# rvaser/rala

Measured on AMD Instinct MI355X. Metric: overlaps/sec (pile build + transitive reduction), higher is better.
Workload: dtype u16/u32 (+f64 compares)

## Files before the change

rala_amd/csrc/context.h:

```cpp
#pragma once

#include <hip/hip_runtime.h>
#include <stdint.h>

#include <algorithm>

#include <memory>
#include <string>
#include <vector>

#include "geom.h"
#include "host_pool.h"
#include "kernels.h"
#include "rala_hip.h"

namespace rala_hip {

struct HostOvl {
    uint32_t src;
    uint32_t a, b;
    Coords c;
    uint8_t strand;
    uint8_t dead;
    uint8_t type;
// ... 145 lines not shown
    hipStream_t side = nullptr;
    hipStream_t aux = nullptr;
    bool use_side_stream = true;
    std::string err;
    hipEvent_t ev[12] = {};
    hipStream_t copy = nullptr;
    hipEvent_t ev_up[4] = {};
    bool upload_pending = false, upload_queued = false;
    const uint32_t* up_src[7] = {};
    const uint8_t* up_strand = nullptr;

    int64_t pool_per_read_x1000 = 1000;
    int64_t max_lds_read_len = 22000;
    int64_t debug_pile_stop_after = 99;
    int64_t host_threads = 0;
    std::unique_ptr<rala_hip::HostPool> pool;
    bool use_run_kernel = true;
    bool debug_fail_construct = false;
    uint32_t debug_pile_variant = 0;
    uint32_t debug_dedupe_list_cap = 0;
    uint32_t debug_fp_lds_limit = 0xFFFFFFFFu;
    bool use_bound_records = true;
    bool use_round_batches = true;
    rala_hip::DevBuf<uint32_t> d_round_log;

    uint64_t n_reads = 0;
    uint32_t max_read_len = 0;
    uint32_t n_class[rala_hip::kPileClasses] = {};
    rala_hip::DevBuf<uint32_t> d_class_order;
    rala_hip::DevBuf<uint32_t> d_seg_base;
    rala_hip::DevBuf<uint32_t> d_dense;
    std::vector<uint32_t> h_read_len;
    std::vector<uint64_t> h_pile_off;
    uint64_t pile_elems = 0;
    rala_hip::DevBuf<uint32_t> d_read_len;
    rala_hip::DevBuf<uint64_t> d_pile_off;
    rala_hip::DevBuf<uint16_t> d_pile;
    rala_hip::DevBuf<uint32_t> d_order, d_overflow;
    rala_hip::DevBuf<uint32_t> d_big_list[2], d_big_space;
    int64_t debug_big_caps = 0;
    bool debug_force_big = false;
    rala_hip::DevBuf<uint16_t> d_slab;
    std::vector<rala_hip::LaunchClass> classes;

    rala_hip::DevBuf<uint8_t> d_name_buckets, d_name_arena, d_paf_text, d_paf_strand;
    uint64_t n_name_buckets = 0;
// ... 145 lines not shown
```

rala_amd/csrc/kernels.h:

```cpp
#pragma once

#include <hip/hip_runtime.h>
#include <stdint.h>

namespace rala_hip {

constexpr uint32_t kPadL = 848;

enum : uint32_t {
    kErrRegionCapacity = 1u,
    kErrPoolCapacity = 2u,
    kErrRawCapacity = 4u,
};

struct Interval {
    uint32_t first, second;
    uint32_t aux;
};

struct PileArgs {
    const uint32_t* read_len;
    const uint64_t* pile_off;
    uint16_t* pile;
    const uint32_t* ev_off;
// ... 222 lines not shown
    const uint32_t* ev_off;
    const uint32_t* ev_cnt;
    uint32_t ev_stride;
    uint32_t ev_shift;
    const uint32_t* sens_off;
    const uint32_t* begin;
    const uint32_t* end;
    uint32_t* out[5];
    uint32_t* counts;
};
void launch_sens_split(const uint32_t* list, uint32_t bound, const uint32_t* n_dev, const SensSplitArgs& args, hipStream_t s);
void launch_status_clear(uint32_t* status, uint32_t bits, uint32_t* zero, hipStream_t s);
void launch_scatter_component_medians(const uint32_t* alive_reads, const uint8_t* touched, const uint16_t* cmed, uint32_t n_alive,
                                      uint16_t* out, hipStream_t s);
void launch_break_hills(const TailReads& R, uint32_t n_reads, hipStream_t s);
void launch_break_pits(const TailReads& R, const uint32_t* alive_reads, const uint8_t* touched, const uint16_t* comp_median,
                       uint32_t n_alive, hipStream_t s, const uint32_t* gate = nullptr);
void launch_retrim(const TailList& L, const TailReads& R, uint32_t promote, uint32_t round, uint32_t* dropped,
                   hipStream_t s, const uint32_t* gate = nullptr);
void launch_cc_edges(const TailList& L, const uint32_t* rank, uint32_t* edges, uint8_t* touched, uint32_t* label, uint32_t n_labels,
                     hipStream_t s);
void launch_refresh_types(const TailList& L, const TailReads& R, hipStream_t s);
hipError_t launch_tail_contain(const TailList& L, const TailReads& R, uint8_t* alive, uint32_t* const lists[6], uint32_t* zeroed21, uint32_t* const work[4],
                               uint32_t* base2, uint8_t* mark2, uint32_t* map, uint32_t* pack, uint32_t n_reads, uint32_t lds_limit, hipStream_t s);
void launch_count_zero_u8(const uint8_t* x, uint32_t n, uint32_t* out, hipStream_t s);
void launch_tail_init(const TailList& L, uint32_t n0, const TailReads& R, uint32_t* n_pits0, uint32_t n_reads, uint32_t* base2,
                      uint8_t* mark2, uint32_t* map, uint32_t* zero22, hipStream_t s);
struct ScanSpace;
bool launch_rank_pass(const uint8_t* alive, uint32_t* rank, uint32_t* alive_reads, uint32_t n_reads, ScanSpace& space, hipStream_t s);
bool launch_node_pass(const uint8_t* alive, uint32_t* node_rank, uint32_t* node_read, uint32_t* n_final, uint32_t n_reads,
                      ScanSpace& space, hipStream_t s);
bool launch_segment_pass(const TailList& L, const TailReads& R, uint32_t want_state, uint32_t want_round, uint32_t* base,
                         uint32_t* next, uint32_t* kept_item, const uint32_t* node_rank, uint32_t* e_src, uint32_t* e_dst,
                         uint32_t* e_len, ScanSpace& space, hipStream_t s);
bool launch_offsets_pass(const uint32_t* in, uint32_t* out, uint32_t* copy, uint32_t n, ScanSpace& space, hipStream_t s);
bool launch_pair_offsets_pass(const uint32_t* in0, const uint32_t* in1, uint32_t* out0, uint32_t* out1, uint32_t* totals, uint32_t n,
                              ScanSpace& space, hipStream_t s);

struct FixedPointList {
    const uint32_t *key, *target, *keeper;
    const uint32_t* count;
    uint32_t lds_limit = 0xFFFFFFFFu;
    uint32_t debug_give_up = 0;
};
size_t fixed_point_pack_words();
hipError_t launch_fixed_point_finish(const FixedPointList& list, uint32_t* base, uint32_t* map, uint32_t* pack, uint32_t* const work[4],
                                     uint32_t* sync8, uint32_t* error, uint32_t* rounds_out, hipStream_t s);

struct FillList {
    static constexpr uint32_t kMost = 8;
    void* ptr[kMost];
    size_t bytes[kMost];
    uint8_t value[kMost];
    uint32_t n = 0;
    bool overflow = false;
    void add(void* p, int byte, size_t n_bytes);
    hipError_t launch(hipStream_t s);
// ... 100 lines not shown
```

rala_amd/csrc/pipeline.hip:

```cpp
#include <hip/hip_runtime.h>
#include <stdio.h>
#include <stdlib.h>
#include <string.h>

#include <algorithm>
#include <chrono>
#include <numeric>

#include "context.h"
#include "scan_pass.h"
#include "stages.h"

using namespace rala_hip;


hipError_t rala_hip::d2h_small(rala_hip_ctx* ctx, void* dst, const void* src, size_t bytes, hipStream_t s) {
    if (ctx->p_stage.ensure(256) != hipSuccess || ctx->stage_used + bytes > 256 * sizeof(uint32_t) ||
        ctx->stage_pending.size() >= 16) {
        return hipMemcpyAsync(dst, src, bytes, hipMemcpyDeviceToHost, s);
    }
    char* at = (char*)ctx->p_stage.p + ctx->stage_used;
    const hipError_t e = hipMemcpyAsync(at, src, bytes, hipMemcpyDeviceToHost, s);
    if (e != hipSuccess) return e;
    ctx->stage_pending.push_back({dst, ctx->stage_used, bytes});
// ... 713 lines not shown
        }
    }
    return true;
}

int materialize_host(rala_hip_ctx* ctx);
int download_repeat_hills(rala_hip_ctx* ctx) {
    if (!ctx->rep_host_stale) return RALA_HIP_OK;
    const uint64_t n = ctx->n_reads;
    HIPCHECK(hipSetDevice(ctx->device));
    ctx->h_n_rep.resize(n); ctx->h_rep_slot.resize(n);
    HIPCHECK(hipMemcpy(ctx->h_n_rep.data(), ctx->d_n_rep.p, n * 4, hipMemcpyDeviceToHost));
    HIPCHECK(hipMemcpy(ctx->h_rep_slot.data(), ctx->d_rep_slot.p, n * 4, hipMemcpyDeviceToHost));
    ctx->h_rep_pool.resize(ctx->n_rep_hills);
    if (ctx->n_rep_hills) {
        HIPCHECK(hipMemcpy(ctx->h_rep_pool.data(), ctx->d_rep_pool.p, (size_t)ctx->n_rep_hills * sizeof(Interval), hipMemcpyDeviceToHost));
    }
    ctx->rep_host_stale = false;
    return RALA_HIP_OK;
}
void build_graph(rala_hip_ctx* ctx);
TailList tail_list(rala_hip_ctx* ctx);
int tail_components(rala_hip_ctx* ctx, const TailList& L, uint32_t n_alive, bool touched_cleared = false);
int gpu_tail_part_b(rala_hip_ctx* ctx);

int preprocess_repeats(rala_hip_ctx* cs, rala_hip_ctx* cl, Comm* comm, const rala_hip_overlaps* sens, uint64_t n_sens,
                       bool device_lists) {
    rala_hip_ctx* ctx = cs;
    const bool sharded = comm != nullptr;
    const uint32_t P = sharded ? comm->world() : 1u, me = sharded ? comm->rank() : 0u;
    const uint64_t n = cs->n_reads;
    const uint64_t nl = cl->n_reads;
    const uint64_t nl_pad = ((n + P - 1) / P + 15) / 16 * 16;
    hipStream_t s = cs->stream;
    hipStream_t sl = cl->stream;
    Trace trc;
    auto comm_fail = [&](const char* what) {
        cs->err = std::string(what) + ": " + comm->error();
        cs->stage_pending.clear();
        cs->stage_used = 0;
        return RALA_HIP_EDEVICE;
    };
    if (n_sens >= 0x7FFFFFF0ull / 2) return fail(ctx, RALA_HIP_EINVAL, "too many sensitive overlaps");
    OvlSoA so;
    {
        const uint32_t* src[7] = {nullptr, nullptr, nullptr, nullptr, nullptr, nullptr, nullptr};
        const uint8_t* dev_strand = nullptr;
// ... 454 lines not shown
}

int tail_components(rala_hip_ctx* ctx, const TailList& L, uint32_t n_alive, bool touched_cleared) {
    hipStream_t s = ctx->stream;
    const uint32_t M = L.n;
    if (!touched_cleared) {
        FillList fills;
        fills.add(ctx->d_touched.p, 0, n_alive);
        component_median_clear(ctx->d_med_tmp.p, n_alive, fills);
        HIPCHECK(fills.launch(s));
    }
    launch_cc_edges(L, ctx->d_rank.p, ctx->d_cc_edges.p, ctx->d_touched.p, ctx->d_cc_label.p, n_alive, s);
    for (int k = 0; k < 2; ++k) {
        launch_cc_hook(ctx->d_cc_edges.p, M, 1, ctx->d_cc_label.p, ctx->d_cc_flags.p + 7, s);
        launch_cc_compress(ctx->d_cc_label.p, n_alive, s);
    }
    launch_cc_hook(ctx->d_cc_edges.p, M, 0, ctx->d_cc_label.p, ctx->d_cc_flags.p + 7, s);
    launch_cc_compress_count(ctx->d_cc_label.p, n_alive, ctx->d_touched.p, component_median_sizes(ctx->d_med_tmp.p, n_alive), s);
    HIPCHECK(launch_component_medians(ctx->d_cc_label.p, ctx->d_touched.p, ctx->d_alive_reads.p, ctx->d_median.p, n_alive,
                                      ctx->d_med_tmp.p, ctx->d_cmed.p, s));
    return RALA_HIP_OK;
}

int gpu_tail_part_a(rala_hip_ctx* ctx) {
    hipStream_t s = ctx->stream;
    Trace trc;
    auto mark = [&](const char* what, size_t k = 0) {
        if (trc.on) { (void)stream_sync(ctx, s); trc(what, k); }
    };
    const uint32_t n_reads = (uint32_t)ctx->n_reads;
    const uint32_t M = ctx->t_n0 + ctx->t_n1;
    const uint32_t n_alive = ctx->t_n_alive;
    const size_t big = (size_t)std::max<uint64_t>(n_reads, M) + 2;
    HIPCHECK(ctx->d_t_state.ensure(M)); HIPCHECK(ctx->d_t_round.ensure(M));
    HIPCHECK(ctx->d_dirty.ensure(n_reads)); HIPCHECK(ctx->d_n_pits0.ensure(n_reads));
    HIPCHECK(ctx->d_rank.ensure(n_reads)); HIPCHECK(ctx->d_alive_reads.ensure(n_reads));
    HIPCHECK(ctx->d_kept_item.ensure(M));
    HIPCHECK(ctx->d_node_rank.ensure(n_reads + 2)); HIPCHECK(ctx->d_t_death[0].ensure(n_reads));
    HIPCHECK(ctx->d_t_death[1].ensure(n_reads));
    HIPCHECK(ctx->d_touched.ensure(n_alive)); HIPCHECK(ctx->d_cmed.ensure(n_alive));
    HIPCHECK(ctx->d_cc_edges.ensure(2 * (size_t)M)); HIPCHECK(ctx->d_cc_label.ensure(n_alive));
    ctx->t_med_tmp = component_median_workspace(n_alive);
    HIPCHECK(ctx->d_med_tmp.ensure(ctx->t_med_tmp));
    HIPCHECK(ctx->d_cc_flags.ensure(8));
    (void)big;
    if ((uint64_t)M >= 0x7FFFFFF0ull) return fail(ctx, RALA_HIP_ETOOLARGE, "too many surviving overlaps");
    const TailList L = tail_list(ctx);
// ... 6 lines not shown
        HIPCHECK(fills.launch(s));
    }
    HIPCHECK(ctx->d_counts.ensure(48));
    for (int k = 0; k < 2; ++k) HIPCHECK(ctx->d_t_work[k].ensure(n_reads));
    HIPCHECK(ctx->d_t_fin.ensure(2 * (size_t)n_reads));
    HIPCHECK(ctx->d_t_mark.ensure(2 * (size_t)n_reads));
    for (int k = 0; k < 3; ++k) { HIPCHECK(ctx->d_kill[k].ensure((size_t)M + 1)); HIPCHECK(ctx->d_kill2[k].ensure((size_t)M + 1)); }
    HIPCHECK(ctx->d_fp_map.ensure(n_reads));
    HIPCHECK(ctx->d_fp_pack.ensure(fixed_point_pack_words()));
    launch_tail_init(L, ctx->t_n0, R, ctx->d_n_pits0.p, n_reads, ctx->d_t_fin.p, ctx->d_t_mark.p, ctx->d_fp_map.p, ctx->d_counts.p + 9, s);
    if (!launch_rank_pass(ctx->d_alive.p, ctx->d_rank.p, ctx->d_alive_reads.p, n_reads, sp, s)) return fail(ctx, RALA_HIP_EDEVICE, "scan space");
    mark("tail: ranks", n_alive);

    HIPCHECK(ctx->d_counts.ensure(48));
    uint32_t* dropped = ctx->d_counts.p + 4;
    launch_break_hills(R, n_reads, s);
    if (ctx->lists_pending) {
        HIPCHECK(hipStreamWaitEvent(s, ctx->ev[3], 0));
        ctx->lists_pending = false;
    }
    launch_retrim(L, R, 0, 0, dropped, s);
    mark("tail: hills + retrim", M);

    uint32_t rounds = 0;
    for (;;) {
        const uint32_t batch = rounds == 0 ? 2u : 1u;
        for (uint32_t k = 0; k < batch; ++k) {
            if (rounds + k >= 255) return fail(ctx, RALA_HIP_EDEVICE, "chimera loop did not settle");
            const uint32_t* gate = k ? dropped + k - 1 : nullptr;
            FillList fills;
            fills.add(ctx->d_dirty.p, 0, n_reads);
            fills.add(ctx->d_touched.p, 0, n_alive);
            component_median_clear(ctx->d_med_tmp.p, n_alive, fills);
            if (k == 0) fills.add(dropped, 0, 2 * 4);
            HIPCHECK(fills.launch(s));
            const int rcc = tail_components(ctx, L, n_alive, true);
            if (rcc != RALA_HIP_OK) return rcc;
            launch_break_pits(R, ctx->d_alive_reads.p, ctx->d_touched.p, ctx->d_cmed.p, n_alive, s, gate);
            launch_retrim(L, R, 1, rounds + k, dropped + k, s, gate);
        }
        uint32_t d[2] = {0, 0};
        HIPCHECK(d2h_small(ctx, d, dropped, sizeof(d), s));
        HIPCHECK(stream_sync(ctx, s));
        mark("tail: pits + retrim", d[0] + d[1]);
        if (!d[0]) { rounds += 1; break; }
        rounds += batch;
        if (!d[batch - 1]) break;
    }
    ctx->t_rounds = rounds;
    if ((uint64_t)M * ((uint64_t)rounds + 2ull) >= 0xFFFFFFF0ull) {
        return fail(ctx, RALA_HIP_ETOOLARGE, "too many surviving overlaps for 32-bit list positions");
    }

    {
        uint32_t* const work[4] = {ctx->d_t_death[0].p, ctx->d_t_death[1].p, ctx->d_t_work[0].p, ctx->d_t_work[1].p};
        uint32_t* const lists[6] = {ctx->d_kill[0].p, ctx->d_kill[1].p, ctx->d_kill[2].p, ctx->d_kill2[0].p, ctx->d_kill2[1].p,
                                    ctx->d_kill2[2].p};
        HIPCHECK(launch_tail_contain(L, R, ctx->d_alive.p, lists, ctx->d_counts.p + 9, work, ctx->d_t_fin.p, ctx->d_t_mark.p, ctx->d_fp_map.p,
                                     ctx->d_fp_pack.p, n_reads, ctx->debug_fp_lds_limit, s));
    }
    mark("tail: containment scans", M);
    return RALA_HIP_OK;
}

int gpu_tail_part_b(rala_hip_ctx* ctx) {
    hipStream_t s = ctx->stream;
    Trace trc;
    auto mark = [&](const char* what, size_t k = 0) {
        if (trc.on) { (void)stream_sync(ctx, s); trc(what, k); }
    };
    const uint32_t n_reads = (uint32_t)ctx->n_reads;
    const uint32_t M = ctx->t_n0 + ctx->t_n1;
    const TailList L = tail_list(ctx);
    const TailReads R = tail_reads(ctx);
    const uint32_t n_seg = ctx->t_rounds + 1;
    HIPCHECK(ctx->d_seg_base.ensure(2 * (size_t)n_seg + 4));
    HIPCHECK(ctx->d_node_read.ensure(2 * (size_t)ctx->t_n_alive + 2));
    for (int k = 0; k < 3; ++k) HIPCHECK(ctx->d_e[k].ensure(2 * (size_t)M + 2));
    HIPCHECK(ctx->d_counts.ensure(48));
    ScanSpace sp;
    {
        FillList fills;
        const int rc = scan_space(ctx, n_seg + 1, std::max<uint64_t>(n_reads, M), sp, &fills);
        if (rc != RALA_HIP_OK) return rc;
        fills.add(ctx->d_seg_base.p, 0, (2 * (size_t)n_seg + 4) * 4);
        fills.add(ctx->d_counts.p + 8, 0, 4);
        HIPCHECK(fills.launch(s));
    }
    if (!launch_node_pass(ctx->d_alive.p, ctx->d_node_rank.p, ctx->d_node_read.p, ctx->d_counts.p + 8, n_reads, sp, s)) {
        return fail(ctx, RALA_HIP_EDEVICE, "scan space");
    }
    for (uint32_t seg = 0; seg < n_seg; ++seg) {
        if (!launch_segment_pass(L, R, seg == 0 ? 1u : 3u, seg == 0 ? 0u : seg - 1, ctx->d_seg_base.p + 2 * seg,
                                 seg + 1 == n_seg ? ctx->d_counts.p + 6 : ctx->d_seg_base.p + 2 * (seg + 1), ctx->d_kept_item.p,
                                 ctx->d_node_rank.p, ctx->d_e[0].p,
                                 ctx->d_e[1].p, ctx->d_e[2].p, sp, s)) {
            return fail(ctx, RALA_HIP_EDEVICE, "scan space");
        }
    }
    uint32_t four[4] = {0, 0, 0, 0};
    HIPCHECK(d2h_small(ctx, four, ctx->d_counts.p + 6, 16, s));
    HIPCHECK(stream_sync(ctx, s));
    const uint32_t totals[2] = {four[0], four[1]}, left[2] = {four[2], four[3]};
    HIPCHECK(hipGetLastError());
    if (getenv("RALA_HIP_TRACE")) {
        uint32_t kc[4] = {0, 0, 0, 0};
        HIPCHECK(hipMemcpy(kc, ctx->d_counts.p + 10, 16, hipMemcpyDeviceToHost));
        fprintf(stderr, "[trace] tail containment killers: %u (%u conditional) among the overlaps, %u (%u) among the internals, of %u items\n",
                kc[0], kc[2], kc[1], kc[3], M);
    }
    if (left[1]) {
        return fail(ctx, RALA_HIP_EDEVICE, "containment fixed point did not converge");
    }
    const uint32_t n_final = left[0];
    ctx->t_n_kept = totals[0];
    ctx->t_n_nodes = 2 * n_final;
    ctx->t_n_edges = 2 * totals[1];
    mark("tail: final list, nodes, edges", ctx->t_n_edges);
    ctx->tail_on_device = true;
    ctx->host_stale = true;
    return RALA_HIP_OK;
}

int gpu_tail_run(rala_hip_ctx* ctx) {
    const int rc = gpu_tail_part_a(ctx);
    return rc != RALA_HIP_OK ? rc : gpu_tail_part_b(ctx);
}

int materialize_host(rala_hip_ctx* ctx) {
    if (ctx->have_repeats && ctx->rep_host_stale) {
        const int rcr = download_repeat_hills(ctx);
        if (rcr != RALA_HIP_OK) return rcr;
    }
    if (!ctx->host_stale) return ctx->host_state_fresh ? RALA_HIP_OK : download_read_state(ctx);
    hipStream_t s = ctx->stream;
    int rc = download_read_state(ctx);
    if (rc != RALA_HIP_OK) return rc;
    const uint32_t M = ctx->t_n0 + ctx->t_n1;
    std::vector<uint32_t> h[8];
    std::vector<uint8_t> strand(M), type(M), state(M);
    for (int f = 0; f < 8; ++f) {
        h[f].resize(M);
        if (M) HIPCHECK(hipMemcpyAsync(h[f].data(), ctx->d_surv_u32[f].p, (size_t)M * 4, hipMemcpyDeviceToHost, s));
    }
    std::vector<uint32_t> kept(ctx->t_n_kept);
    if (M) {
        HIPCHECK(hipMemcpyAsync(strand.data(), ctx->d_surv_u8[0].p, M, hipMemcpyDeviceToHost, s));
        HIPCHECK(hipMemcpyAsync(type.data(), ctx->d_surv_u8[1].p, M, hipMemcpyDeviceToHost, s));
        HIPCHECK(hipMemcpyAsync(state.data(), ctx->d_t_state.p, M, hipMemcpyDeviceToHost, s));
// ... 502 lines not shown
    if (ctx->stream) (void)hipStreamSynchronize(ctx->stream);
    if (ctx->side) (void)hipStreamSynchronize(ctx->side);
    if (ctx->aux) (void)hipStreamSynchronize(ctx->aux);
    for (auto& e : ctx->ev) if (e) (void)hipEventDestroy(e);
    for (auto& e : ctx->ev_up) if (e) (void)hipEventDestroy(e);
    if (ctx->copy) (void)hipStreamDestroy(ctx->copy);
    if (ctx->side) (void)hipStreamDestroy(ctx->side);
    if (ctx->aux) (void)hipStreamDestroy(ctx->aux);
    if (ctx->stream) (void)hipStreamDestroy(ctx->stream);
    delete ctx;
}

const char* rala_hip_last_error(const rala_hip_ctx* ctx) { return ctx ? ctx->err.c_str() : "no context"; }

int rala_hip_set_option(rala_hip_ctx* ctx, const char* key, int64_t value) {
    if (!ctx || !key) return RALA_HIP_EINVAL;
    if (!strcmp(key, "interval_pool_per_read_x1000")) { ctx->pool_per_read_x1000 = value; return RALA_HIP_OK; }
    if (!strcmp(key, "debug_big_caps")) { ctx->debug_big_caps = value; return RALA_HIP_OK; }
    if (!strcmp(key, "debug_force_big")) { ctx->debug_force_big = value != 0; return RALA_HIP_OK; }
    if (!strcmp(key, "max_lds_read_len")) { ctx->max_lds_read_len = value; return RALA_HIP_OK; }
    if (!strcmp(key, "debug_pile_stop_after")) { ctx->debug_pile_stop_after = value; return RALA_HIP_OK; }
    if (!strcmp(key, "use_run_kernel")) { ctx->use_run_kernel = value != 0; return RALA_HIP_OK; }
    if (!strcmp(key, "use_round_batches")) { ctx->use_round_batches = value != 0; return RALA_HIP_OK; }
    if (!strcmp(key, "use_bound_records")) { ctx->use_bound_records = value != 0; return RALA_HIP_OK; }
    if (!strcmp(key, "use_fused_emit")) { ctx->use_fused_emit = value != 0; return RALA_HIP_OK; }
    if (!strcmp(key, "ingest_window_bytes")) { ctx->ingest_window_bytes = std::max<int64_t>(0, value); return RALA_HIP_OK; }
    if (!strcmp(key, "pile_chunk_mb")) { ctx->pile_chunk_mb = (uint32_t)std::max<int64_t>(0, std::min<int64_t>(value, 1 << 20)); return RALA_HIP_OK; }
    if (!strcmp(key, "debug_ev_events")) { ctx->debug_ev_events = value != 0; return RALA_HIP_OK; }
    if (!strcmp(key, "debug_count_window")) { g_count_window = (uint32_t)std::max<int64_t>(0, value); return RALA_HIP_OK; }
    if (!strcmp(key, "debug_part_shift")) { g_part_shift = (uint32_t)std::max<int64_t>(0, value); return RALA_HIP_OK; }
    if (!strcmp(key, "debug_pile_variant")) { ctx->debug_pile_variant = (uint32_t)std::max<int64_t>(0, value); return RALA_HIP_OK; }
    if (!strcmp(key, "debug_dedupe_list_cap")) { ctx->debug_dedupe_list_cap = (uint32_t)std::max<int64_t>(0, value); return RALA_HIP_OK; }
    if (!strcmp(key, "debug_fp_lds_limit")) { ctx->debug_fp_lds_limit = (uint32_t)std::max<int64_t>(0, value); return RALA_HIP_OK; }
    if (!strcmp(key, "debug_fail_construct")) { ctx->debug_fail_construct = value != 0; return RALA_HIP_OK; }
    if (!strcmp(key, "use_gpu_tail")) { ctx->use_gpu_tail = value != 0; return RALA_HIP_OK; }
    if (!strcmp(key, "use_fixed_buckets")) { ctx->use_fixed_buckets = value != 0; return RALA_HIP_OK; }
    if (!strcmp(key, "use_partitioned_buckets")) { ctx->use_partitioned_buckets = value != 0; return RALA_HIP_OK; }
    if (!strcmp(key, "use_side_stream")) { ctx->use_side_stream = value != 0; return RALA_HIP_OK; }
    if (!strcmp(key, "sensitive_in_device_memory")) { ctx->sens_in_device = value != 0; return RALA_HIP_OK; }
    if (!strcmp(key, "host_threads")) {
        ctx->host_threads = value;
        ctx->pool.reset(new HostPool((unsigned)std::max<int64_t>(1, std::min<int64_t>(value, 256))));
        return RALA_HIP_OK;
    }
    return fail(ctx, RALA_HIP_EINVAL, "unknown option");
}
// ... 1115 lines not shown
```

rala_amd/csrc/scan_pass.h:

```cpp
#pragma once

#include <hip/hip_runtime.h>
#include <stdint.h>

#include "device_utils.h"

namespace rala_hip {

constexpr uint32_t kScanBlock = 256;
constexpr uint32_t kScanItems = 8;
constexpr uint32_t kScanTile = kScanBlock * kScanItems;

constexpr uint64_t kScanValueMask = (1ull << 62) - 1ull;
constexpr uint64_t kScanAggregate = 1ull << 62;
constexpr uint64_t kScanPrefix = 2ull << 62;

inline uint32_t scan_tiles_for(uint64_t n) { return (uint32_t)((n + kScanTile - 1) / kScanTile); }

template <class F>
__global__ __launch_bounds__(kScanBlock) void scan_pass_kernel(uint32_t n, F f, uint64_t* __restrict__ state, uint32_t* ticket) {
    __shared__ uint64_t tmp[kScanBlock / 64 + 1];
    __shared__ uint32_t s_tile;
    __shared__ uint64_t s_before;
    const uint32_t n_tiles = (n + kScanTile - 1) / kScanTile;
    if (threadIdx.x == 0) {
        const uint32_t t = atomicAdd(ticket, 1u);
        s_tile = t;
        if (t + 1 == n_tiles) *ticket = 0;
    }
    __syncthreads();
    const uint32_t tile = s_tile;
    uint64_t v[kScanItems], ex[kScanItems];
    uint64_t tile_sum = 0;
#pragma unroll
    for (uint32_t k = 0; k < kScanItems; ++k) {
        const uint32_t i = tile * kScanTile + k * kScanBlock + threadIdx.x;
        v[k] = i < n ? f.value(i) : 0ull;
    }
#pragma unroll
    for (uint32_t k = 0; k < kScanItems; ++k) {
        uint64_t tot;
        ex[k] = tile_sum + block_scan_excl<(int)kScanBlock>(v[k], OpAdd(), (uint64_t)0, tmp, tot);
        tile_sum += tot;
    }
    if (threadIdx.x < 64) {
        const uint32_t lane = threadIdx.x;
// ... 27 lines not shown
    }
    __syncthreads();
    const uint64_t before = s_before;
#pragma unroll
    for (uint32_t k = 0; k < kScanItems; ++k) {
        const uint32_t i = tile * kScanTile + k * kScanBlock + threadIdx.x;
        if (i < n) f.place(i, v[k], before + ex[k]);
    }
}

struct ScanSpace {
    uint64_t* state = nullptr;
    uint32_t* ticket = nullptr;
    size_t words = 0, used = 0;
    uint64_t* take(uint64_t n_items) {
        const size_t need = scan_tiles_for(n_items) + 1;
        uint64_t* p = state + used;
        used += need;
        return used <= words ? p : nullptr;
    }
};

template <class F>
inline bool launch_scan_pass(uint32_t n, const F& f, ScanSpace& space, hipStream_t s) {
    if (n == 0) return true;
    uint64_t* st = space.take(n);
    if (!st) return false;
    hipLaunchKernelGGL(scan_pass_kernel<F>, dim3(scan_tiles_for(n)), dim3(kScanBlock), 0, s, n, f, st, space.ticket);
    return true;
}

}
```

rala_amd/csrc/tail_kernels.hip:

```cpp
#include <hip/hip_runtime.h>

#include <algorithm>

#include "device_utils.h"
#include "geom.h"
#include "kernels.h"
#include "scan_pass.h"

namespace rala_hip {

namespace {

constexpr int kBlock = 256;
constexpr uint32_t kInf = 0xFFFFFFFFu;

inline dim3 grid_for(uint64_t n) { return dim3((unsigned)((n + kBlock - 1) / kBlock)); }

__device__ __forceinline__ bool dev_shrink(const TailReads& R, uint32_t r, uint32_t b, uint32_t e) {
    if (b > e || e - b < kMinRegion) { R.dirty[r] = 1; return false; }
    if (R.begin[r] != b || R.end[r] != e) R.dirty[r] = 1;
    R.begin[r] = b;
    R.end[r] = e;
    return true;
}
// ... 121 lines not shown

struct BlockAppend {
    uint32_t* s_cnt;
    uint32_t* s_base;
    __device__ uint32_t note(bool mine) const {
        const uint32_t lane = threadIdx.x & 63u;
        const uint64_t m = __ballot(mine);
        uint32_t base = 0;
        if (m) {
            const uint32_t leader = (uint32_t)__ffsll((long long)m) - 1u;
            if (lane == leader) base = atomicAdd(s_cnt, (uint32_t)__popcll(m));
            base = (uint32_t)__shfl((int)base, (int)leader);
        }
        return mine ? base + (uint32_t)__popcll(m & ((1ull << lane) - 1ull)) : kInf;
    }
    __device__ void reserve(uint32_t* counter) const {
        __syncthreads();
        if (threadIdx.x == 0) *s_base = *s_cnt ? atomicAdd(counter, *s_cnt) : 0u;
        __syncthreads();
    }
};

__global__ __launch_bounds__(kContainBlock) void tail_contain_collect_kernel(TailList L, TailReads R, const uint8_t* __restrict__ alive,
                                                                             TailKillers K) {
    __shared__ uint32_t s_cnt[2], s_base[2];
    if (threadIdx.x < 2) s_cnt[threadIdx.x] = 0;
    __syncthreads();
    const BlockAppend app[2] = {{&s_cnt[0], &s_base[0]}, {&s_cnt[1], &s_base[1]}};
    uint32_t key[kCollectPer], target[kCollectPer], keeper[kCollectPer], slot[kCollectPer], cls[kCollectPer];
#pragma unroll
    for (uint32_t u = 0; u < kCollectPer; ++u) {
        const uint32_t k = (blockIdx.x * kCollectPer + u) * kContainBlock + threadIdx.x;
        bool killer = false;
        cls[u] = 0; key[u] = 0; target[u] = 0; keeper[u] = 0;
        if (k < L.n) {
            const uint8_t st = L.state[k];
            uint8_t t = L.type[k];
            if (st != 0 && t == 255) {
                const uint32_t a = L.a[k], b = L.b[k];
                if (alive[a] && alive[b]) {
                    const Coords c = item_coords(L, k);
                    t = (uint8_t)ovl_type(c, L.strand[k], R.begin[a], R.end[a], R.begin[b], R.end[b]);
                    L.type[k] = t;
                }
            }
            if (st != 0 && (t == kTypeA || t == kTypeB)) {
                const uint32_t a = L.a[k], b = L.b[k];
// ... 38 lines not shown
        uint32_t key = 0, target = 0, keeper = 0;
        if (i < n) {
            const uint32_t at = kClass ? n_items - 1u - i : i;
            key = K.key[at]; target = K.target[at]; keeper = K.keeper[at];
            const bool ok = kClass == 0 || !(gone_before_second_scan(alive, K.base[0], target) ||
                                             gone_before_second_scan(alive, K.base[0], keeper));
            if (ok) {
                if (K.mark[kClass][keeper]) conditional = true;
                else if (ld_past_l1(base + target) > key) atomicMin(base + target, key);
            }
        }
        const uint32_t slot = app.note(conditional);
        app.reserve(&K.count[2 + kClass]);
        if (conditional) {
            const uint32_t w = s_base + slot;
            K.c_key[w] = key; K.c_target[w] = target; K.c_keeper[w] = keeper;
        }
        __syncthreads();
    }
}

__global__ __launch_bounds__(kBlock) void tail_contain_apply_kernel(TailList L, const uint8_t* __restrict__ alive,
                                                                    const uint32_t* __restrict__ base0,
                                                                    const uint32_t* __restrict__ base1) {
    const uint32_t k = blockIdx.x * kBlock + threadIdx.x;
    if (k >= L.n) return;
    const uint8_t st = L.state[k];
    if (st == 0) return;
    const uint8_t t = L.type[k];
    bool drop = t == kTypeA || t == kTypeB;
    if (st == 2 && !drop) {
        const uint32_t a = L.a[k], b = L.b[k];
        drop = gone_before_second_scan(alive, base0, a) || gone_before_second_scan(alive, base0, b) || base1[a] < k || base1[b] < k;
    }
    if (drop) L.state[k] = 0;
}

__global__ __launch_bounds__(kBlock) void tail_contain_kill_kernel(TailKillers K, uint32_t n_items, uint8_t* alive) {
    const uint32_t n0 = K.count[0], n1 = K.count[1];
    for (uint32_t i = blockIdx.x * kBlock + threadIdx.x; i < n0 + n1; i += gridDim.x * kBlock) {
        const uint32_t target = K.target[i < n0 ? i : n_items - 1u - (i - n0)];
        if (K.base[0][target] != kInf || K.base[1][target] != kInf) alive[target] = 0;
    }
}

__global__ __launch_bounds__(kBlock) void tail_init_kernel(uint8_t* state, uint8_t* round, uint32_t n0, uint32_t m,
                                                           uint8_t* dirty, uint32_t* n_pits0, const uint32_t* n_pits,
// ... 113 lines not shown
void launch_break_hills(const TailReads& R, uint32_t n_reads, hipStream_t s) {
    if (n_reads) hipLaunchKernelGGL(break_hills_kernel, grid_for(n_reads), dim3(kBlock), 0, s, R, n_reads);
}
void launch_break_pits(const TailReads& R, const uint32_t* alive_reads, const uint8_t* touched, const uint16_t* comp_median,
                       uint32_t n_alive, hipStream_t s, const uint32_t* gate) {
    if (n_alive) {
        hipLaunchKernelGGL(break_pits_kernel, grid_for(n_alive), dim3(kBlock), 0, s, R, alive_reads, touched, comp_median,
                           n_alive, gate);
    }
}
void launch_retrim(const TailList& L, const TailReads& R, uint32_t promote, uint32_t round, uint32_t* dropped,
                   hipStream_t s, const uint32_t* gate) {
    if (L.n) hipLaunchKernelGGL(retrim_kernel, grid_for(L.n), dim3(kBlock), 0, s, L, R, promote, round, dropped, gate);
}
void launch_cc_edges(const TailList& L, const uint32_t* rank, uint32_t* edges, uint8_t* touched, uint32_t* label, uint32_t n_labels,
                     hipStream_t s) {
    const uint32_t n = std::max<uint32_t>(L.n, n_labels);
    if (n) hipLaunchKernelGGL(cc_edges_kernel, grid_for(n), dim3(kBlock), 0, s, L, rank, edges, touched, label, n_labels);
}
void launch_refresh_types(const TailList& L, const TailReads& R, hipStream_t s) {
    if (L.n) hipLaunchKernelGGL(refresh_types_kernel, grid_for(L.n), dim3(kBlock), 0, s, L, R);
}
hipError_t launch_tail_contain(const TailList& L, const TailReads& R, uint8_t* alive, uint32_t* const lists[6], uint32_t* zeroed21, uint32_t* const work[4],
                               uint32_t* base2, uint8_t* mark2, uint32_t* map, uint32_t* pack, uint32_t n_reads, uint32_t lds_limit, hipStream_t s) {
    if (!L.n) return hipSuccess;
    TailKillers K;
    K.key = lists[0]; K.target = lists[1]; K.keeper = lists[2];
    K.c_key = lists[3]; K.c_target = lists[4]; K.c_keeper = lists[5];
    K.error = zeroed21; K.count = zeroed21 + 1;
    K.mark[0] = mark2; K.mark[1] = mark2 + n_reads;
    K.base[0] = base2; K.base[1] = base2 + n_reads;
    const uint32_t per_block = kCollectPer * kContainBlock;
    hipLaunchKernelGGL(tail_contain_collect_kernel, dim3((L.n + per_block - 1) / per_block), dim3(kContainBlock), 0, s, L, R,
                       (const uint8_t*)alive, K);
    for (int c = 0; c < 2; ++c) {
        if (c == 0) hipLaunchKernelGGL(tail_contain_reduce_kernel<0>, dim3(128), dim3(kBlock), 0, s, K, L.n, (const uint8_t*)alive);
        else hipLaunchKernelGGL(tail_contain_reduce_kernel<1>, dim3(128), dim3(kBlock), 0, s, K, L.n, (const uint8_t*)alive);
        const FixedPointList conditional = {K.c_key, K.c_target, K.c_keeper, K.count + 2 + c, lds_limit};
        const hipError_t e = launch_fixed_point_finish(conditional, K.base[c], map, pack, work, zeroed21 + 5 + 8 * c, K.error, nullptr, s);
        if (e != hipSuccess) return e;
    }
    hipLaunchKernelGGL(tail_contain_apply_kernel, grid_for(L.n), dim3(kBlock), 0, s, L, (const uint8_t*)alive,
                       (const uint32_t*)K.base[0], (const uint32_t*)K.base[1]);
    hipLaunchKernelGGL(tail_contain_kill_kernel, dim3(128), dim3(kBlock), 0, s, K, L.n, alive);
    return hipGetLastError();
}
void launch_tail_init(const TailList& L, uint32_t n0, const TailReads& R, uint32_t* n_pits0, uint32_t n_reads, uint32_t* base2,
                      uint8_t* mark2, uint32_t* map, uint32_t* zero22, hipStream_t s) {
    const uint32_t n = std::max<uint32_t>(std::max<uint32_t>(L.n, n_reads), 22u);
    hipLaunchKernelGGL(tail_init_kernel, grid_for(n), dim3(kBlock), 0, s, L.state, L.round, n0, L.n, R.dirty, n_pits0, R.n_pits, n_reads,
                       base2, mark2, map, zero22);
}
bool launch_rank_pass(const uint8_t* alive, uint32_t* rank, uint32_t* alive_reads, uint32_t n_reads, ScanSpace& space, hipStream_t s) {
    return launch_scan_pass(n_reads, RankPass{alive, rank, alive_reads}, space, s);
}
bool launch_node_pass(const uint8_t* alive, uint32_t* node_rank, uint32_t* node_read, uint32_t* n_final, uint32_t n_reads,
                      ScanSpace& space, hipStream_t s) {
    return launch_scan_pass(n_reads, NodePass{alive, node_rank, node_read, n_final}, space, s);
}
bool launch_segment_pass(const TailList& L, const TailReads& R, uint32_t want_state, uint32_t want_round, uint32_t* base,
                         uint32_t* next, uint32_t* kept_item, const uint32_t* node_rank, uint32_t* e_src, uint32_t* e_dst,
                         uint32_t* e_len, ScanSpace& space, hipStream_t s) {
    SegmentPass f;
    f.L = L; f.R = R; f.want_state = want_state; f.want_round = want_round; f.base = base; f.kept_item = kept_item;
    f.node_rank = node_rank; f.e_src = e_src; f.e_dst = e_dst; f.e_len = e_len; f.next = next;
    return launch_scan_pass(L.n, f, space, s);
}
bool launch_pair_offsets_pass(const uint32_t* in0, const uint32_t* in1, uint32_t* out0, uint32_t* out1, uint32_t* totals, uint32_t n,
                              ScanSpace& space, hipStream_t s) {
    return launch_scan_pass(n, PairOffsetsPass{in0, in1, out0, out1, totals, n}, space, s);
}
bool launch_offsets_pass(const uint32_t* in, uint32_t* out, uint32_t* copy, uint32_t n, ScanSpace& space, hipStream_t s) {
    return launch_scan_pass(n, OffsetsPass{in, out, copy, n}, space, s);
}

namespace {
__global__ __launch_bounds__(256) void count_zero_u8_kernel(const uint8_t* __restrict__ x, uint32_t n, uint32_t* out) {
    const uint32_t i = blockIdx.x * 256 + threadIdx.x;
    const uint64_t m = __ballot(i < n && x[i] == 0);
    if (m && (threadIdx.x & 63) == 0) atomicAdd(out, (uint32_t)__popcll(m));
}
}
void launch_count_zero_u8(const uint8_t* x, uint32_t n, uint32_t* out, hipStream_t s) {
    if (n) hipLaunchKernelGGL(count_zero_u8_kernel, dim3((n + 255) / 256), dim3(256), 0, s, x, n, out);
}

}
```

Measured before the change: 7.196 billion.

## Run containment and graph build speculatively ahead of chimera loop convergence

Instead of syncing on the host after the first chimera rounds before launching containment and graph segmentation, the code now enqueues two chimera rounds, containment, node pass and segment passes back to back. Device-side gates (hold and run_if_set flags read from the dropped counters) turn the speculative kernels into no-ops when a round still dropped reads. A single host readback then checks convergence and falls back to the full loop plus a rebuild if needed. This removes one or more host round-trips on the common path, at the cost of wasted launches and a redo when the loop does not settle within two rounds.

```diff
diff --git a/rala_amd/csrc/context.h b/rala_amd/csrc/context.h
--- a/rala_amd/csrc/context.h
+++ b/rala_amd/csrc/context.h
@@ -191,6 +191,7 @@
     uint32_t debug_fp_lds_limit = 0xFFFFFFFFu;
     bool use_bound_records = true;
     bool use_round_batches = true;
+    uint32_t tail_ahead_rounds = 2;
     rala_hip::DevBuf<uint32_t> d_round_log;
 
     uint64_t n_reads = 0;
diff --git a/rala_amd/csrc/kernels.h b/rala_amd/csrc/kernels.h
--- a/rala_amd/csrc/kernels.h
+++ b/rala_amd/csrc/kernels.h
@@ -268,17 +268,19 @@
                      hipStream_t s);
 void launch_refresh_types(const TailList& L, const TailReads& R, hipStream_t s);
 hipError_t launch_tail_contain(const TailList& L, const TailReads& R, uint8_t* alive, uint32_t* const lists[6], uint32_t* zeroed21, uint32_t* const work[4],
-                               uint32_t* base2, uint8_t* mark2, uint32_t* map, uint32_t* pack, uint32_t n_reads, uint32_t lds_limit, hipStream_t s);
+                               uint32_t* base2, uint8_t* mark2, uint32_t* map, uint32_t* pack, uint32_t n_reads, uint32_t lds_limit, hipStream_t s,
+                               const uint32_t* hold = nullptr);
 void launch_count_zero_u8(const uint8_t* x, uint32_t n, uint32_t* out, hipStream_t s);
 void launch_tail_init(const TailList& L, uint32_t n0, const TailReads& R, uint32_t* n_pits0, uint32_t n_reads, uint32_t* base2,
                       uint8_t* mark2, uint32_t* map, uint32_t* zero22, hipStream_t s);
 struct ScanSpace;
 bool launch_rank_pass(const uint8_t* alive, uint32_t* rank, uint32_t* alive_reads, uint32_t n_reads, ScanSpace& space, hipStream_t s);
 bool launch_node_pass(const uint8_t* alive, uint32_t* node_rank, uint32_t* node_read, uint32_t* n_final, uint32_t n_reads,
-                      ScanSpace& space, hipStream_t s);
+                      ScanSpace& space, hipStream_t s, const uint32_t* run_if_zero = nullptr);
 bool launch_segment_pass(const TailList& L, const TailReads& R, uint32_t want_state, uint32_t want_round, uint32_t* base,
                          uint32_t* next, uint32_t* kept_item, const uint32_t* node_rank, uint32_t* e_src, uint32_t* e_dst,
-                         uint32_t* e_len, ScanSpace& space, hipStream_t s);
+                         uint32_t* e_len, ScanSpace& space, hipStream_t s, const uint32_t* run_if_zero = nullptr,
+                         const uint32_t* run_if_set = nullptr);
 bool launch_offsets_pass(const uint32_t* in, uint32_t* out, uint32_t* copy, uint32_t n, ScanSpace& space, hipStream_t s);
 bool launch_pair_offsets_pass(const uint32_t* in0, const uint32_t* in1, uint32_t* out0, uint32_t* out1, uint32_t* totals, uint32_t n,
                               ScanSpace& space, hipStream_t s);
diff --git a/rala_amd/csrc/pipeline.hip b/rala_amd/csrc/pipeline.hip
--- a/rala_amd/csrc/pipeline.hip
+++ b/rala_amd/csrc/pipeline.hip
@@ -759,7 +759,7 @@
 void build_graph(rala_hip_ctx* ctx);
 TailList tail_list(rala_hip_ctx* ctx);
 int tail_components(rala_hip_ctx* ctx, const TailList& L, uint32_t n_alive, bool touched_cleared = false);
-int gpu_tail_part_b(rala_hip_ctx* ctx);
+int gpu_tail_part_b(rala_hip_ctx* ctx, bool ahead = false);
 
 int preprocess_repeats(rala_hip_ctx* cs, rala_hip_ctx* cl, Comm* comm, const rala_hip_overlaps* sens, uint64_t n_sens,
                        bool device_lists) {
@@ -1260,7 +1260,63 @@
     return RALA_HIP_OK;
 }
 
-int gpu_tail_part_a(rala_hip_ctx* ctx) {
+constexpr uint32_t kAheadRounds = 2;
+
+int chimera_round(rala_hip_ctx* ctx, const TailList& L, const TailReads& R, uint32_t round, uint32_t k) {
+    hipStream_t s = ctx->stream;
+    const uint32_t n_alive = ctx->t_n_alive;
+    uint32_t* dropped = ctx->d_counts.p + 4;
+    if (round >= 255) return fail(ctx, RALA_HIP_EDEVICE, "chimera loop did not settle");
+    const uint32_t* gate = k ? dropped + k - 1 : nullptr;
+    FillList fills;
+    fills.add(ctx->d_dirty.p, 0, ctx->n_reads);
+    fills.add(ctx->d_touched.p, 0, n_alive);
+    component_median_clear(ctx->d_med_tmp.p, n_alive, fills);
+    if (k == 0) fills.add(dropped, 0, kAheadRounds * 4);
+    HIPCHECK(fills.launch(s));
+    const int rcc = tail_components(ctx, L, n_alive, true);
+    if (rcc != RALA_HIP_OK) return rcc;
+    launch_break_pits(R, ctx->d_alive_reads.p, ctx->d_touched.p, ctx->d_cmed.p, n_alive, s, gate);
+    launch_retrim(L, R, 1, round, dropped + k, s, gate);
+    return RALA_HIP_OK;
+}
+
+int chimera_loop(rala_hip_ctx* ctx, const TailList& L, const TailReads& R, uint32_t rounds) {
+    hipStream_t s = ctx->stream;
+    Trace trc;
+    const uint32_t* dropped = ctx->d_counts.p + 4;
+    for (;;) {
+        const uint32_t batch = rounds == 0 ? kAheadRounds : 1u;
+        for (uint32_t k = 0; k < batch; ++k) {
+            const int rc = chimera_round(ctx, L, R, rounds + k, k);
+            if (rc != RALA_HIP_OK) return rc;
+        }
+        uint32_t d[kAheadRounds] = {};
+        HIPCHECK(d2h_small(ctx, d, dropped, sizeof(d), s));
+        HIPCHECK(stream_sync(ctx, s));
+        if (trc.on) trc("tail: pits + retrim", d[0] + d[1]);
+        uint32_t k = 0;
+        while (k + 1 < batch && d[k]) ++k;
+        rounds += k + 1;
+        if (!d[k]) break;
+    }
+    ctx->t_rounds = rounds;
+    if ((uint64_t)(ctx->t_n0 + ctx->t_n1) * ((uint64_t)rounds + 2ull) >= 0xFFFFFFF0ull) {
+        return fail(ctx, RALA_HIP_ETOOLARGE, "too many surviving overlaps for 32-bit list positions");
+    }
+    return RALA_HIP_OK;
+}
+
+int tail_contain(rala_hip_ctx* ctx, const TailList& L, const TailReads& R, const uint32_t* hold) {
+    uint32_t* const work[4] = {ctx->d_t_death[0].p, ctx->d_t_death[1].p, ctx->d_t_work[0].p, ctx->d_t_work[1].p};
+    uint32_t* const lists[6] = {ctx->d_kill[0].p, ctx->d_kill[1].p, ctx->d_kill[2].p, ctx->d_kill2[0].p, ctx->d_kill2[1].p,
+                                ctx->d_kill2[2].p};
+    HIPCHECK(launch_tail_contain(L, R, ctx->d_alive.p, lists, ctx->d_counts.p + 9, work, ctx->d_t_fin.p, ctx->d_t_mark.p, ctx->d_fp_map.p,
+                                 ctx->d_fp_pack.p, (uint32_t)ctx->n_reads, ctx->debug_fp_lds_limit, ctx->stream, hold));
+    return RALA_HIP_OK;
+}
+
+int gpu_tail_part_a(rala_hip_ctx* ctx, bool* graph_ahead = nullptr) {
     hipStream_t s = ctx->stream;
     Trace trc;
     auto mark = [&](const char* what, size_t k = 0) {
@@ -1313,48 +1369,30 @@
     launch_retrim(L, R, 0, 0, dropped, s);
     mark("tail: hills + retrim", M);
 
-    uint32_t rounds = 0;
-    for (;;) {
-        const uint32_t batch = rounds == 0 ? 2u : 1u;
-        for (uint32_t k = 0; k < batch; ++k) {
-            if (rounds + k >= 255) return fail(ctx, RALA_HIP_EDEVICE, "chimera loop did not settle");
-            const uint32_t* gate = k ? dropped + k - 1 : nullptr;
-            FillList fills;
-            fills.add(ctx->d_dirty.p, 0, n_reads);
-            fills.add(ctx->d_touched.p, 0, n_alive);
-            component_median_clear(ctx->d_med_tmp.p, n_alive, fills);
-            if (k == 0) fills.add(dropped, 0, 2 * 4);
-            HIPCHECK(fills.launch(s));
-            const int rcc = tail_components(ctx, L, n_alive, true);
-            if (rcc != RALA_HIP_OK) return rcc;
-            launch_break_pits(R, ctx->d_alive_reads.p, ctx->d_touched.p, ctx->d_cmed.p, n_alive, s, gate);
-            launch_retrim(L, R, 1, rounds + k, dropped + k, s, gate);
-        }
-        uint32_t d[2] = {0, 0};
-        HIPCHECK(d2h_small(ctx, d, dropped, sizeof(d), s));
-        HIPCHECK(stream_sync(ctx, s));
-        mark("tail: pits + retrim", d[0] + d[1]);
-        if (!d[0]) { rounds += 1; break; }
-        rounds += batch;
-        if (!d[batch - 1]) break;
-    }
-    ctx->t_rounds = rounds;
-    if ((uint64_t)M * ((uint64_t)rounds + 2ull) >= 0xFFFFFFF0ull) {
-        return fail(ctx, RALA_HIP_ETOOLARGE, "too many surviving overlaps for 32-bit list positions");
-    }
-
+    const uint32_t ahead = std::min(ctx->tail_ahead_rounds, kAheadRounds);
+    if (graph_ahead && ahead && (uint64_t)M * (ahead + 2ull) < 0xFFFFFFF0ull) {
+        for (uint32_t k = 0; k < ahead; ++k) {
+            const int rc = chimera_round(ctx, L, R, k, k);
+            if (rc != RALA_HIP_OK) return rc;
+        }
+        ctx->t_rounds = ahead;
+        *graph_ahead = true;
+        return tail_contain(ctx, L, R, dropped + ahead - 1);
+    }
+    if (graph_ahead) *graph_ahead = false;
     {
-        uint32_t* const work[4] = {ctx->d_t_death[0].p, ctx->d_t_death[1].p, ctx->d_t_work[0].p, ctx->d_t_work[1].p};
-        uint32_t* const lists[6] = {ctx->d_kill[0].p, ctx->d_kill[1].p, ctx->d_kill[2].p, ctx->d_kill2[0].p, ctx->d_kill2[1].p,
-                                    ctx->d_kill2[2].p};
-        HIPCHECK(launch_tail_contain(L, R, ctx->d_alive.p, lists, ctx->d_counts.p + 9, work, ctx->d_t_fin.p, ctx->d_t_mark.p, ctx->d_fp_map.p,
-                                     ctx->d_fp_pack.p, n_reads, ctx->debug_fp_lds_limit, s));
+        const int rc = chimera_loop(ctx, L, R, 0);
+        if (rc != RALA_HIP_OK) return rc;
+    }
+    {
+        const int rc = tail_contain(ctx, L, R, nullptr);
+        if (rc != RALA_HIP_OK) return rc;
     }
     mark("tail: containment scans", M);
     return RALA_HIP_OK;
 }
 
-int gpu_tail_part_b(rala_hip_ctx* ctx) {
+int gpu_tail_part_b(rala_hip_ctx* ctx, bool ahead) {
     hipStream_t s = ctx->stream;
     Trace trc;
     auto mark = [&](const char* what, size_t k = 0) {
@@ -1365,6 +1403,8 @@
     const TailList L = tail_list(ctx);
     const TailReads R = tail_reads(ctx);
     const uint32_t n_seg = ctx->t_rounds + 1;
+    const uint32_t* dropped = ctx->d_counts.p + 4;
+    const uint32_t* hold = ahead ? dropped + ctx->t_rounds - 1 : nullptr;
     HIPCHECK(ctx->d_seg_base.ensure(2 * (size_t)n_seg + 4));
     HIPCHECK(ctx->d_node_read.ensure(2 * (size_t)ctx->t_n_alive + 2));
     for (int k = 0; k < 3; ++k) HIPCHECK(ctx->d_e[k].ensure(2 * (size_t)M + 2));
@@ -1378,22 +1418,33 @@
         fills.add(ctx->d_counts.p + 8, 0, 4);
         HIPCHECK(fills.launch(s));
     }
-    if (!launch_node_pass(ctx->d_alive.p, ctx->d_node_rank.p, ctx->d_node_read.p, ctx->d_counts.p + 8, n_reads, sp, s)) {
+    if (!launch_node_pass(ctx->d_alive.p, ctx->d_node_rank.p, ctx->d_node_read.p, ctx->d_counts.p + 8, n_reads, sp, s, hold)) {
         return fail(ctx, RALA_HIP_EDEVICE, "scan space");
     }
     for (uint32_t seg = 0; seg < n_seg; ++seg) {
         if (!launch_segment_pass(L, R, seg == 0 ? 1u : 3u, seg == 0 ? 0u : seg - 1, ctx->d_seg_base.p + 2 * seg,
                                  seg + 1 == n_seg ? ctx->d_counts.p + 6 : ctx->d_seg_base.p + 2 * (seg + 1), ctx->d_kept_item.p,
                                  ctx->d_node_rank.p, ctx->d_e[0].p,
-                                 ctx->d_e[1].p, ctx->d_e[2].p, sp, s)) {
+                                 ctx->d_e[1].p, ctx->d_e[2].p, sp, s, hold, ahead && seg >= 2 ? dropped + seg - 2 : nullptr)) {
             return fail(ctx, RALA_HIP_EDEVICE, "scan space");
         }
     }
-    uint32_t four[4] = {0, 0, 0, 0};
-    HIPCHECK(d2h_small(ctx, four, ctx->d_counts.p + 6, 16, s));
+    uint32_t six[6] = {0, 0, 0, 0, 0, 0};
+    HIPCHECK(d2h_small(ctx, six, ctx->d_counts.p + 4, 24, s));
     HIPCHECK(stream_sync(ctx, s));
-    const uint32_t totals[2] = {four[0], four[1]}, left[2] = {four[2], four[3]};
+    const uint32_t totals[2] = {six[2], six[3]}, left[2] = {six[4], six[5]};
     HIPCHECK(hipGetLastError());
+    if (ahead) {
+        const uint32_t batch = ctx->t_rounds;
+        if (six[batch - 1]) {
+            int rc = chimera_loop(ctx, L, R, batch);
+            if (rc == RALA_HIP_OK) rc = tail_contain(ctx, L, R, nullptr);
+            return rc != RALA_HIP_OK ? rc : gpu_tail_part_b(ctx, false);
+        }
+        uint32_t rounds = 1;
+        while (rounds < batch && six[rounds - 1]) ++rounds;
+        ctx->t_rounds = rounds;
+    }
     if (getenv("RALA_HIP_TRACE")) {
         uint32_t kc[4] = {0, 0, 0, 0};
         HIPCHECK(hipMemcpy(kc, ctx->d_counts.p + 10, 16, hipMemcpyDeviceToHost));
@@ -1414,8 +1465,9 @@
 }
 
 int gpu_tail_run(rala_hip_ctx* ctx) {
-    const int rc = gpu_tail_part_a(ctx);
-    return rc != RALA_HIP_OK ? rc : gpu_tail_part_b(ctx);
+    bool ahead = false;
+    const int rc = gpu_tail_part_a(ctx, &ahead);
+    return rc != RALA_HIP_OK ? rc : gpu_tail_part_b(ctx, ahead);
 }
 
 int materialize_host(rala_hip_ctx* ctx) {
@@ -1964,6 +2016,7 @@
     if (!strcmp(key, "debug_pile_stop_after")) { ctx->debug_pile_stop_after = value; return RALA_HIP_OK; }
     if (!strcmp(key, "use_run_kernel")) { ctx->use_run_kernel = value != 0; return RALA_HIP_OK; }
     if (!strcmp(key, "use_round_batches")) { ctx->use_round_batches = value != 0; return RALA_HIP_OK; }
+    if (!strcmp(key, "tail_ahead_rounds")) { ctx->tail_ahead_rounds = (uint32_t)std::max<int64_t>(0, std::min<int64_t>(value, 2)); return RALA_HIP_OK; }
     if (!strcmp(key, "use_bound_records")) { ctx->use_bound_records = value != 0; return RALA_HIP_OK; }
     if (!strcmp(key, "use_fused_emit")) { ctx->use_fused_emit = value != 0; return RALA_HIP_OK; }
     if (!strcmp(key, "ingest_window_bytes")) { ctx->ingest_window_bytes = std::max<int64_t>(0, value); return RALA_HIP_OK; }
diff --git a/rala_amd/csrc/scan_pass.h b/rala_amd/csrc/scan_pass.h
--- a/rala_amd/csrc/scan_pass.h
+++ b/rala_amd/csrc/scan_pass.h
@@ -17,11 +17,22 @@
 
 inline uint32_t scan_tiles_for(uint64_t n) { return (uint32_t)((n + kScanTile - 1) / kScanTile); }
 
+struct ScanGate {
+    const uint32_t* run_if_zero = nullptr;
+    const uint32_t* run_if_set = nullptr;
+    __device__ bool holds() const { return (run_if_zero && *run_if_zero != 0) || (run_if_set && *run_if_set == 0); }
+};
+
 template <class F>
-__global__ __launch_bounds__(kScanBlock) void scan_pass_kernel(uint32_t n, F f, uint64_t* __restrict__ state, uint32_t* ticket) {
+__global__ __launch_bounds__(kScanBlock) void scan_pass_kernel(uint32_t n, F f, uint64_t* __restrict__ state, uint32_t* ticket,
+                                                               ScanGate gate) {
     __shared__ uint64_t tmp[kScanBlock / 64 + 1];
     __shared__ uint32_t s_tile;
     __shared__ uint64_t s_before;
+    if (gate.holds()) {
+        if (blockIdx.x == 0 && threadIdx.x == 0) f.total(0ull);
+        return;
+    }
     const uint32_t n_tiles = (n + kScanTile - 1) / kScanTile;
     if (threadIdx.x == 0) {
         const uint32_t t = atomicAdd(ticket, 1u);
@@ -95,11 +106,11 @@
 };
 
 template <class F>
-inline bool launch_scan_pass(uint32_t n, const F& f, ScanSpace& space, hipStream_t s) {
+inline bool launch_scan_pass(uint32_t n, const F& f, ScanSpace& space, hipStream_t s, ScanGate gate = ScanGate()) {
     if (n == 0) return true;
     uint64_t* st = space.take(n);
     if (!st) return false;
-    hipLaunchKernelGGL(scan_pass_kernel<F>, dim3(scan_tiles_for(n)), dim3(kScanBlock), 0, s, n, f, st, space.ticket);
+    hipLaunchKernelGGL(scan_pass_kernel<F>, dim3(scan_tiles_for(n)), dim3(kScanBlock), 0, s, n, f, st, space.ticket, gate);
     return true;
 }
 
diff --git a/rala_amd/csrc/tail_kernels.hip b/rala_amd/csrc/tail_kernels.hip
--- a/rala_amd/csrc/tail_kernels.hip
+++ b/rala_amd/csrc/tail_kernels.hip
@@ -167,7 +167,8 @@
 };
 
 __global__ __launch_bounds__(kContainBlock) void tail_contain_collect_kernel(TailList L, TailReads R, const uint8_t* __restrict__ alive,
-                                                                             TailKillers K) {
+                                                                             TailKillers K, const uint32_t* hold) {
+    if (hold && *hold != 0) return;
     __shared__ uint32_t s_cnt[2], s_base[2];
     if (threadIdx.x < 2) s_cnt[threadIdx.x] = 0;
     __syncthreads();
@@ -252,7 +253,8 @@
 
 __global__ __launch_bounds__(kBlock) void tail_contain_apply_kernel(TailList L, const uint8_t* __restrict__ alive,
                                                                     const uint32_t* __restrict__ base0,
-                                                                    const uint32_t* __restrict__ base1) {
+                                                                    const uint32_t* __restrict__ base1, const uint32_t* hold) {
+    if (hold && *hold != 0) return;
     const uint32_t k = blockIdx.x * kBlock + threadIdx.x;
     if (k >= L.n) return;
     const uint8_t st = L.state[k];
@@ -412,7 +414,8 @@
     if (L.n) hipLaunchKernelGGL(refresh_types_kernel, grid_for(L.n), dim3(kBlock), 0, s, L, R);
 }
 hipError_t launch_tail_contain(const TailList& L, const TailReads& R, uint8_t* alive, uint32_t* const lists[6], uint32_t* zeroed21, uint32_t* const work[4],
-                               uint32_t* base2, uint8_t* mark2, uint32_t* map, uint32_t* pack, uint32_t n_reads, uint32_t lds_limit, hipStream_t s) {
+                               uint32_t* base2, uint8_t* mark2, uint32_t* map, uint32_t* pack, uint32_t n_reads, uint32_t lds_limit, hipStream_t s,
+                               const uint32_t* hold) {
     if (!L.n) return hipSuccess;
     TailKillers K;
     K.key = lists[0]; K.target = lists[1]; K.keeper = lists[2];
@@ -422,7 +425,7 @@
     K.base[0] = base2; K.base[1] = base2 + n_reads;
     const uint32_t per_block = kCollectPer * kContainBlock;
     hipLaunchKernelGGL(tail_contain_collect_kernel, dim3((L.n + per_block - 1) / per_block), dim3(kContainBlock), 0, s, L, R,
-                       (const uint8_t*)alive, K);
+                       (const uint8_t*)alive, K, hold);
     for (int c = 0; c < 2; ++c) {
         if (c == 0) hipLaunchKernelGGL(tail_contain_reduce_kernel<0>, dim3(128), dim3(kBlock), 0, s, K, L.n, (const uint8_t*)alive);
         else hipLaunchKernelGGL(tail_contain_reduce_kernel<1>, dim3(128), dim3(kBlock), 0, s, K, L.n, (const uint8_t*)alive);
@@ -431,7 +434,7 @@
         if (e != hipSuccess) return e;
     }
     hipLaunchKernelGGL(tail_contain_apply_kernel, grid_for(L.n), dim3(kBlock), 0, s, L, (const uint8_t*)alive,
-                       (const uint32_t*)K.base[0], (const uint32_t*)K.base[1]);
+                       (const uint32_t*)K.base[0], (const uint32_t*)K.base[1], hold);
     hipLaunchKernelGGL(tail_contain_kill_kernel, dim3(128), dim3(kBlock), 0, s, K, L.n, alive);
     return hipGetLastError();
 }
@@ -445,16 +448,21 @@
     return launch_scan_pass(n_reads, RankPass{alive, rank, alive_reads}, space, s);
 }
 bool launch_node_pass(const uint8_t* alive, uint32_t* node_rank, uint32_t* node_read, uint32_t* n_final, uint32_t n_reads,
-                      ScanSpace& space, hipStream_t s) {
-    return launch_scan_pass(n_reads, NodePass{alive, node_rank, node_read, n_final}, space, s);
+                      ScanSpace& space, hipStream_t s, const uint32_t* run_if_zero) {
+    ScanGate gate;
+    gate.run_if_zero = run_if_zero;
+    return launch_scan_pass(n_reads, NodePass{alive, node_rank, node_read, n_final}, space, s, gate);
 }
 bool launch_segment_pass(const TailList& L, const TailReads& R, uint32_t want_state, uint32_t want_round, uint32_t* base,
                          uint32_t* next, uint32_t* kept_item, const uint32_t* node_rank, uint32_t* e_src, uint32_t* e_dst,
-                         uint32_t* e_len, ScanSpace& space, hipStream_t s) {
+                         uint32_t* e_len, ScanSpace& space, hipStream_t s, const uint32_t* run_if_zero, const uint32_t* run_if_set) {
     SegmentPass f;
     f.L = L; f.R = R; f.want_state = want_state; f.want_round = want_round; f.base = base; f.kept_item = kept_item;
     f.node_rank = node_rank; f.e_src = e_src; f.e_dst = e_dst; f.e_len = e_len; f.next = next;
-    return launch_scan_pass(L.n, f, space, s);
+    ScanGate gate;
+    gate.run_if_zero = run_if_zero;
+    gate.run_if_set = run_if_set;
+    return launch_scan_pass(L.n, f, space, s, gate);
 }
 bool launch_pair_offsets_pass(const uint32_t* in0, const uint32_t* in1, uint32_t* out0, uint32_t* out1, uint32_t* totals, uint32_t n,
                               ScanSpace& space, hipStream_t s) {
```

Measured after the change: 7.256 billion (median of 6 runs). Within noise of the previous version (+0.8%).
